# talmolab/flybody

Measured on AMD Instinct MI355X. Metric: env-steps/sec (whole node), fruitfly flight-imitation task, higher is better.
Workload: dtype f32; 1 GPU; flight_imitation (BASELINE configs[3]): 4 substeps @5e-5 s (joint limits, fluid forces, the fly's own contacts) + WBPG + obs/reward/termination/auto-reset; envs_per_gpu=8192, global_batch=8192, parallelism=env-sharded x1, actions=uniform over the raw action spec (canonical U(-1,1)), resident in HBM

## Files before the change

### flybody_amd/build.py

```python

from __future__ import annotations

import os
import subprocess

_HERE = os.path.dirname(os.path.abspath(__file__))
CSRC = os.path.join(_HERE, "csrc")
LIB = os.path.join(CSRC, "libflybody_env.so")
SOURCES = ["fly_env.hip", "ball_env.hip", "nstep.hip"]
PER_SOURCE_FLAGS = {
    "fly_env.hip": ["-mllvm", "-disable-machine-licm"],
    "ball_env.hip": ["-mllvm", "-sink-insts-to-avoid-spills=1"],
}
HEADERS = ["dev_model.hpp", "ball_model.hpp", "ball_env.hpp", "dev_math.hpp", "convex.hpp", "launch_order.hpp", os.path.join("..", "..", "include", "flybody_env.h")]


def needs_build() -> bool:
    if not os.path.exists(LIB):
        return True
    t = os.path.getmtime(LIB)
    return any(os.path.getmtime(os.path.join(CSRC, f)) > t for f in SOURCES + HEADERS)


def _common_flags() -> list:
    hipcc = os.environ.get("HIPCC", "/opt/rocm/bin/hipcc")
    common = [hipcc, "--offload-arch=gfx950", "-O3", "-std=c++17", "-fPIC", "-fno-slp-vectorize",
              "-mllvm", "-amdgpu-sched-strategy=iterative-ilp"]
    return common


def kernel_resource_usage(src: str = "fly_env.hip", match: str = "flight_step_kernel") -> dict:
    import re
    import tempfile

    with tempfile.TemporaryDirectory() as tmp:
        cmd = _common_flags() + PER_SOURCE_FLAGS.get(src, []) + ["--cuda-device-only", "-Rpass-analysis=kernel-resource-usage", "-c",
                                                                 os.path.join(CSRC, src), "-o", os.path.join(tmp, "dev.o")]
        text = subprocess.run(cmd, check=True, stderr=subprocess.PIPE, stdout=subprocess.DEVNULL, text=True).stderr
    out, cur = {}, None
    for line in text.splitlines():
        m = re.search(r"remark: Function Name: (\S+)", line)
        if m:
            cur = out.setdefault(m.group(1), {}) if match in m.group(1) else None
            continue
        m = re.search(r"remark:\s+([A-Za-z ]+?)(?: \[[^\]]*\])?: (\d+)", line)
        if m and cur is not None:
            cur[m.group(1).strip()] = int(m.group(2))
    return out


def build(force: bool = False, verbose: bool = False) -> str:
    if not force and not needs_build():
        return LIB
    common = _common_flags()
    hipcc = common[0]
    objs = []
    for src in SOURCES:
        obj = os.path.join(CSRC, "_obj_" + os.path.splitext(src)[0] + ".o")
        cmd = common + PER_SOURCE_FLAGS.get(src, []) + ["-c", os.path.join(CSRC, src), "-o", obj]
        if verbose:
            print(" ".join(cmd))
        subprocess.check_call(cmd)
        objs.append(obj)
    cmd = [hipcc, "--offload-arch=gfx950", "-shared", "-fPIC", "-o", LIB] + objs
    if verbose:
        print(" ".join(cmd))
    subprocess.check_call(cmd)
    for obj in objs:
        os.remove(obj)
    return LIB


if __name__ == "__main__":
    print(build(force=True, verbose=True))
```

### flybody_amd/csrc/fly_env.hip

```cpp
#include <hip/hip_runtime.h>

#include <cstdio>
#include <cstring>
#include <memory>
#include <string>
#include <vector>

#include "../../include/flybody_env.h"
#include "ball_env.hpp"
#include "dev_model.hpp"
#include "launch_order.hpp"
#include "dev_math.hpp"
#include "convex.hpp"

#ifndef FFE_WAVES_PER_SIMD
#define FFE_WAVES_PER_SIMD 4
#endif

namespace ffe {

constexpr int kMC = 6;
constexpr int kMCX = 12;
constexpr int kCapExit = 0x100;
constexpr int kNSD = 16;
// ... 325 lines not shown
  } while (0)
#endif
#ifdef FFE_DBGCF
__device__ float g_dbgcf[64][4 + 6 * 12];
#endif
#ifdef FFE_STAMPS
__device__ unsigned long long g_stamps[20];
#define STAMP_DECL unsigned long long st_t0 = __builtin_amdgcn_s_memtime(), st_acc[20] = {0}
#define STAMP(k)                                                   \
  do {                                                             \
    __builtin_amdgcn_s_waitcnt(0);                                 \
    unsigned long long st_t1 = __builtin_amdgcn_s_memtime();       \
    c.st_acc[k] += st_t1 - c.st_t0;                                \
    c.st_t0 = st_t1;                                               \
  } while (0)
#define CSTAMP(k)                                                                                  \
  do {                                                                                             \
    __builtin_amdgcn_s_waitcnt(0);                                                                 \
    unsigned long long cs_t1 = __builtin_amdgcn_s_memtime();                                       \
    if (lane == 0) atomicAdd(&g_stamps[k], cs_t1 - cs_t0);                                         \
    cs_t0 = cs_t1;                                                                                 \
  } while (0)
#define CSTAMP_DECL unsigned long long cs_t0 = __builtin_amdgcn_s_memtime()
#else
#define STAMP(k) do {} while (0)
#define CSTAMP(k) do {} while (0)
#define CSTAMP_DECL do {} while (0)
#endif
__device__ __forceinline__ void set_com(Ctx &c, V3 v) { if (c.lane == 0) { c.T.sens[9] = v.x; c.T.sens[10] = v.y; c.T.sens[11] = v.z; } }
__device__ __forceinline__ V3 get_com(const Ctx &c) { return {c.T.sens[9], c.T.sens[10], c.T.sens[11]}; }
#ifdef FFE_TRACE
#define TRACE_HI(c) (((unsigned)(c).nrare & 0xffu) | (((unsigned)(c).nfac & 0xffu) << 8) | ((min((c).tr_coll, 0xffffu)) << 16))
__device__ unsigned long long g_trace[32768][4];
#define TRACE_BEGIN unsigned long long tr_t0 = __builtin_amdgcn_s_memrealtime(); const int tr_prev = cost[order[blockIdx.x]]
#define TRACE_END(slot, tr_extra, tr_hi)                                                                                              \
  do {                                                                                                                         \
    __builtin_amdgcn_s_waitcnt(0);                                                                                             \
    if (threadIdx.x == 0 && (slot) < 32768) {                                                                                  \
      g_trace[slot][0] = tr_t0; g_trace[slot][1] = __builtin_amdgcn_s_memrealtime();                                               \
      g_trace[slot][2] = (unsigned long long)__builtin_amdgcn_s_getreg((31 << 11) | 4) | ((unsigned long long)tr_hi << 32);                                                 \
      g_trace[slot][3] = (__builtin_amdgcn_s_getreg((31 << 11) | 20) & 0xf) | ((unsigned long long)(tr_extra) << 8);  \
    }                                                                                                                          \
  } while (0)
#else
#define TRACE_BEGIN do {} while (0)
#define TRACE_HI(c) 0
#define TRACE_END(slot, tr_extra, tr_hi) do {} while (0)
#endif
#ifdef FFE_ABLATION
#define DBG(c, f) ((c).flags & (f))
#else
#define DBG(c, f) (0)
#endif
enum { DBG_SKIP_FACTOR = 1 << 16, DBG_SKIP_SOLVE = 1 << 17, DBG_SKIP_STAGE1 = 1 << 18, DBG_SKIP_MENTRIES = 1 << 19, DBG_SKIP_GHOST = 1 << 20, DBG_SKIP_WBPG = 1 << 21, DBG_SKIP_OBS = 1 << 22, DBG_NO_CARRY = 1 << 23, DBG_NO_ORDER = 1 << 24 };

struct CollA { float4 gc[kMaxGeom], gq[kMaxGeom]; float lq[kMaxLink][4]; float sdc[kNSD][5], sdn[kNSD][5]; };
constexpr int kCL2 = 24;
template <int MC> struct CollB { unsigned short cl1[128], cl2[kCL2]; float rec[MC][12]; float cl2n[kCL2][5]; };
static_assert(sizeof(CollA) <= sizeof(Tile::LD), "collision scratch A");
static_assert(sizeof(CollB<kMC>) == 1072 && sizeof(CollB<kMCX>) == 1360 && sizeof(CollB<kMCX>) <= sizeof(Tile::lT) + sizeof(Tile::lb) + sizeof(Tile::lc) && offsetof(Tile, lc) == offsetof(Tile, lT) + sizeof(Tile::lT) + sizeof(Tile::lb), "collision scratch B");
__device__ __forceinline__ CollA &coll_a(Tile &T) { return *reinterpret_cast<CollA *>(&T.LD[0]); }
template <int MC> __device__ __forceinline__ CollB<MC> &coll_b(Tile &T) { return *reinterpret_cast<CollB<MC> *>(&T.lT[0][0]); }

__device__ __forceinline__ cvx::Geom load_geom(const CollA &A, const DevModel FFE_CONST &M, int g) {
  const float4 cc = A.gc[g], qq = A.gq[g];
  return cvx::Geom{dm::V3{cc.x, cc.y, cc.z}, dm::Q4{qq.x, qq.y, qq.z, qq.w}, M.cg_size[g], M.cg_size[kMaxGeom + g], M.cg_size[2 * kMaxGeom + g], M.cg_type[g]};
}

__device__ __forceinline__ cvx::UShape ush(const DevModel FFE_CONST &M, int g) {
  const float4 u = M.cg_ush[2 * g], k = M.cg_ush[2 * g + 1];
  return cvx::UShape{u.x, u.y, u.z, u.w, k.x, k.y, k.z, k.w};
}

template <bool WITH_RARE, int MC>
__device__ __forceinline__ int collide_narrow(Tile &T, const DevModel FFE_CONST &M, const int lane, int n2, int nk, int ovf) {
  CollA &A = coll_a(T);
  CollB<MC> &B = coll_b<MC>(T);
  const unsigned long long mm0 = M.cg_mmask[0], mm1 = M.cg_mmask[1];
  const float mclass = M.c_margin;
  auto pair_margin = [&](int a, int b) {
    const bool ma = a < 64 ? ((mm0 >> a) & 1ull) : ((mm1 >> (a - 64)) & 1ull), mb = b < 64 ? ((mm0 >> b) & 1ull) : ((mm1 >> (b - 64)) & 1ull);
    return (ma || mb) ? mclass : 0.f;
  };
  bool hit = false;
  float dist = 0.f, margin = 0.f, ctt = 0.f;
  dm::V3 nrm = {1.f, 0.f, 0.f}, cpos = {0.f, 0.f, 0.f};
  int a = 0, b = 0;
// ... 987 lines not shown
    obs[L.gyro] = s_gyro.x; obs[L.gyro + 1] = s_gyro.y; obs[L.gyro + 2] = s_gyro.z;
    obs[L.vel] = s_vel.x; obs[L.vel + 1] = s_vel.y; obs[L.vel + 2] = s_vel.z;
    obs[L.zaxis] = T.xmat[0][6]; obs[L.zaxis + 1] = T.xmat[0][7]; obs[L.zaxis + 2] = T.xmat[0][8];
  }
  if (lane < M.nobsj) {
    obs[L.jpos + lane] = T.qpos[M.obsj_qadr[lane]];
    obs[L.jvel + lane] = T.qvel[M.obsj_dof[lane]];
  }
  float cd = 0.f;
  Q4 r0 = {1.f, 0.f, 0.f, 0.f};
  if (lane < nref) {
    const double *r = K.ref_qpos + ((size_t)traj_row0 + step_counter + lane) * 7;
    V3 dv = {(float)(r[0] - T.rootpos[0]), (float)(r[1] - T.rootpos[1]), (float)(r[2] - T.rootpos[2])};
    V3 e = mtv(ldm(T.xmat[0]), dv);
    obs[L.rdisp + 3 * lane] = e.x; obs[L.rdisp + 3 * lane + 1] = e.y; obs[L.rdisp + 3 * lane + 2] = e.z;
    Q4 fq = {T.qpos[3], T.qpos[4], T.qpos[5], T.qpos[6]};
    Q4 dq = qmul(quat_recip(fq), Q4{(float)r[3], (float)r[4], (float)r[5], (float)r[6]});
    obs[L.rquat + 4 * lane] = dq.w; obs[L.rquat + 4 * lane + 1] = dq.x; obs[L.rquat + 4 * lane + 2] = dq.y; obs[L.rquat + 4 * lane + 3] = dq.z;
    if (lane == 0) { cd = sqrtf(dot(e, e)); r0 = dq; }
  }
  com_dist = __shfl(cd, 0);
  rq0 = {__shfl(r0.w, 0), __shfl(r0.x, 0), __shfl(r0.y, 0), __shfl(r0.z, 0)};
}

__device__ __forceinline__ void load_lane_consts(Ctx &c) {
  const DevModel FFE_CONST &M = *c.Mp;
  c.dinv[0] = c.dinv[1] = 0.f;
  c.la_pack = (unsigned)M.d_madr[c.lane] | ((unsigned)M.d_depth[c.lane] << 10) | ((unsigned)M.d_ndesc[c.lane] << 16);
  c.seq0 = M.br_seq[c.lane]; c.seq1 = M.br_seq[kWave + c.lane]; c.seq2 = M.br_seq[2 * kWave + c.lane]; c.seq3 = M.br_seq[3 * kWave + c.lane];
  for (int e = c.lane; e < M.nM; e += kWave) c.T.colmadr[e] = M.colmadr[e];
}

template <int MC>
__global__ __launch_bounds__(kWave, FFE_WAVES_PER_SIMD) void flight_step_kernel(const DevModel *__restrict__ Mp_, const TaskDev *__restrict__ Kp_, typename StateOf<MC>::type *__restrict__ states, const float *__restrict__ act,
                                                              float *__restrict__ obs_out, float *__restrict__ reward_out,
                                                              float *__restrict__ discount_out, int *__restrict__ step_type_out, int batch, int mode, int nphys,
                                                              const int *__restrict__ order, int *__restrict__ cost,
                                                              const unsigned char *__restrict__ reset_mask) {
  __shared__ Tile T;
  const DevModel FFE_CONST *Mp = (const DevModel FFE_CONST *)Mp_;
  const TaskDev FFE_CONST *Kp = (const TaskDev FFE_CONST *)Kp_;
  const DevModel FFE_CONST &M = *Mp;
  const TaskDev FFE_CONST &K = *Kp;
  if ((int)blockIdx.x >= batch) return;
  TRACE_BEGIN;
  const int env = order[blockIdx.x];
  if (mode == 3) {
    if (!reset_mask[env]) return;
    mode = 1;
  }
  const int lane = threadIdx.x;
  typename StateOf<MC>::type &SX = states[env];
  EnvState &S = common(SX);
  Ctx c{Mp, T, lane, K.flags, 0.f, 0.f, {0.f, 0.f}, 0u, 0u, 0u, 0u, 0u};
#ifdef FFE_DBGCF
  c.dbg_env = env;
#endif
  c.pc = -1;
  c.nrare = 0; c.nfac = 0;
#ifdef FFE_TRACE
  c.tr_coll = 0u;
#endif
#ifdef FFE_STAMPS
  c.st_t0 = __builtin_amdgcn_s_memtime();
  for (int k = 0; k < 20; k++) c.st_acc[k] = 0;
#endif
  load_lane_consts(c);
  if (lane < kNSD) { c.sd_nx = S.sd_n[lane][0]; c.sd_ny = S.sd_n[lane][1]; c.sd_nz = S.sd_n[lane][2]; c.sd_t = S.sd_n[lane][3]; c.sd_pid = S.sd_pid[lane]; }
  c.sd_cnt = S.s1_valid ? S.sd_cnt : 0;
  float *obs = obs_out + (size_t)env * K.obs_dim;
  const bool phys_only = (mode == 2);
  const int nsub = phys_only ? nphys : M.nsub;

  if (lane < 3) T.rootpos[lane] = S.rootpos[lane];
  if (lane < 9) T.sens[lane] = 0.f;
  unsigned long long lo_mask = S.lo_mask, hi_mask = S.hi_mask, in_lo = S.in_lo_mask, in_hi = S.in_hi_mask;
  int wb_step = S.wb_step, wb_idx = S.wb_freq_idx, step_counter = S.step_counter, traj_idx = S.traj_idx;
  double wb_cf = S.wb_ctrl_freq;
  int wb_off = S.wb_off, wb_len = S.wb_len, traj_row0 = S.traj_row0;
  const bool do_reset = !phys_only && ((mode == 1) || (S.needs_reset != 0));
  int iters = 0;
  const bool have_saved = !do_reset && S.s1_valid != 0 && !DBG(c, DBG_NO_CARRY);
  constexpr int kCarry = (kMaxDof * 6 + kWave - 1) / kWave;
  float pre_c[kCarry], pre_b[kCarry], pre_f = 0.f, pre_m = 0.f;
  if (have_saved) {
#pragma unroll
    for (int k = 0; k < kCarry; k++) {
      const int e = lane + k * kWave;
      pre_c[k] = e < kMaxDof * 6 ? S.s1_cdof[e] : 0.f; pre_b[k] = e < kMaxDof * 6 ? S.s1_buf[e] : 0.f;
    }
    pre_f = S.s1_f[lane];
    pre_m = lane < 12 ? S.s1_misc[lane] : 0.f;
  }

  unsigned long long episode = S.episode;
  float ctrl_reg = 0.f;
  if (do_reset) {
    double phase;
    if (S.forced_traj >= 0) { traj_idx = S.forced_traj; phase = S.forced_phase; }
    else {
      traj_idx = (int)(env_rng(K.seed, K.env_id_base + env, episode, 0) % (unsigned long long)K.ntraj);
      phase = (double)(env_rng(K.seed, K.env_id_base + env, episode, 1) >> 11) * (1.0 / 9007199254740992.0);
    }
    episode++;
    step_counter = 0;
    wb_cf = K.base_freq;
    wb_idx = wave_argmin_absdiff(K.beat_freqs, K.nfreq, wb_cf, lane);
    int off = K.tab_off[wb_idx], len = K.tab_off[wb_idx + 1] - off;
    wb_off = off; wb_len = len;
    wb_step = wave_argmin_absdiff(K.phase + off, len, phase, lane);
    const int nxt = wb_step + 1 < len ? wb_step + 1 : 0;
    const int row0 = K.traj_off[traj_idx];
    traj_row0 = row0;
    const double *rq = K.ref_qpos + (size_t)row0 * 7, *rv = K.ref_qvel + (size_t)row0 * 6;
    if (lane < kMaxDof + 4) { T.qpos[lane] = lane < M.nq ? M.qpos0[lane] : 0.f; T.qvel[lane] = 0.f; }
    SYNC();
    if (lane == 0) {
// ... 41 lines not shown
                                             : wave_argmin_absdiff(K.beat_freqs, K.nfreq, wb_cf, lane));
      if (idx_new != wb_idx) {
        double cur = K.phase_frac[wb_off + wb_step];
        int noff = K.tab_off[idx_new], nlen = K.tab_off[idx_new + 1] - noff;
        wb_step = wave_argmin_absdiff(K.phase_frac + noff, nlen, cur, lane);
        wb_idx = idx_new; wb_off = noff; wb_len = nlen;
        if (lane < M.nwing) tgt = K.traj[(size_t)(wb_off + wb_step) * 6 + lane];
      }
    }
    STAMP(15);
    if (lane < M.nu) T.ctrl[lane] = ai >= 0 ? to_real(a_raw, ai) : 0.f;
    if (lane < 13) T.ghost[lane] = gh;
    SYNC();
    if (lane < M.nwing) {
      float add = tgt - T.qpos[M.wing_qadr[lane]];
      const int u = M.wing_ctrl[lane];
      if (u >= 0) T.ctrl[u] += add;
    }
    SYNC();
    ctrl_reg = lane < M.nu ? T.ctrl[lane] : 0.f;
    SYNC();
    step_counter++;
  }
  {
    const float abase = do_reset ? 0.f : actuation_base(c, ctrl_reg);
    if (lane < kMaxAct) T.ctrl[lane] = abase;
  }
  if (lane == 0) {
    T.park_d[0] = wb_cf; T.park_d[1] = __longlong_as_double((long long)episode);
    T.park_i[0] = wb_step; T.park_i[1] = wb_idx; T.park_i[2] = step_counter; T.park_i[3] = traj_idx; T.park_i[4] = 0; T.park_i[5] = 0;
    T.park_i[6] = S.v_ep_flagged; T.park_i[7] = S.v_ep_bits;
  }
  STAMP(11);
  const int nst = do_reset ? 1 : nsub;
#pragma unroll 1
  for (int s = 0; s <= nst; s++) {
    if (s == 0 && have_saved) {
#pragma unroll
      for (int k = 0; k < kCarry; k++) {
        const int e = lane + k * kWave;
        if (e < kMaxDof * 6) { (&T.cdof[0][0])[e] = pre_c[k]; (&T.buf[0][0])[e] = pre_b[k]; }
      }
      c.f_smooth_nb = pre_f;
      if (lane < MC) {
        const float *o = ct_f_row(SX, lane);
        c.ct_nx = o[0]; c.ct_ny = o[1]; c.ct_nz = o[2]; c.ct_px = o[3]; c.ct_py = o[4]; c.ct_pz = o[5]; c.ct_dist = o[6]; c.ct_incl = o[7]; c.ct_invw = o[8];
        const int *oi = ct_i_row(SX, lane);
        c.ct_l1 = oi[0]; c.ct_l2 = oi[1]; c.ct_pid = oi[2];
      }
      c.nct = S.nct;
      if (lane < 9) T.xmat[0][lane] = pre_m;
      else if (lane < 12) T.sens[lane] = pre_m;
      SYNC();
    } else if (!DBG(c, DBG_SKIP_STAGE1) || s == 0) { stage1(c); flight_collide<MC>(c); STAMP(16); }
    if (lane < 6 && (do_reset || s > 0)) {
      float add;
      if (lane < 3) add = T.xmat[0][lane] * T.qvel[0] + T.xmat[0][3 + lane] * T.qvel[1] + T.xmat[0][6 + lane] * T.qvel[2];
      else add = T.qvel[lane];
      T.sens[lane < 3 ? 6 + lane : lane] += add;
    }
    if (s == nst) break;
    float qa = 0.f;
    if (!do_reset) qa = actuation(c, lane < kMaxAct ? T.ctrl[lane] : 0.f);
    STAMP(12);
    int it = 0;
    const V3 acc = stage2<MC>(c, qa, !do_reset, !do_reset && !phys_only && !DBG(c, DBG_SKIP_GHOST), K.ghost_accel_z, lo_mask, hi_mask, in_lo, in_hi, it);
    if (lane == 0) { T.park_i[4] += it; if (s < 4) T.park_i[5] |= min(c.nct, 15) << (4 * s); }
    if (lane < 3) T.sens[lane] += lane == 0 ? acc.x : (lane == 1 ? acc.y : acc.z);
    if (do_reset) break;
  }
  SYNC();
  wb_cf = T.park_d[0]; episode = (unsigned long long)__double_as_longlong(T.park_d[1]);
  wb_step = T.park_i[0]; wb_idx = T.park_i[1]; step_counter = T.park_i[2]; traj_idx = T.park_i[3]; iters = T.park_i[4];
  V3 s_acc = {T.sens[0], T.sens[1], T.sens[2]}, s_gyro = {T.sens[3], T.sens[4], T.sens[5]}, s_vel = {T.sens[6], T.sens[7], T.sens[8]};
  if (!phys_only) {
  const float inv = (do_reset && K.pad_first_obs) ? 1.f : 1.f / (float)nsub;
  float cdist;
  Q4 rq0;
  const int traj_row0 = K.traj_off[traj_idx], traj_rows = K.traj_off[traj_idx + 1] - traj_row0;
  if (DBG(c, DBG_SKIP_OBS)) { cdist = 0.f; rq0 = {1.f, 0.f, 0.f, 0.f}; }
  else write_obs(c, K, obs, inv * s_acc, inv * s_gyro, inv * s_vel, traj_row0, step_counter, cdist, rq0);
  if (do_reset) {
    if (lane == 0) { reward_out[env] = 0.f; discount_out[env] = 1.f; step_type_out[env] = FFE_STEP_FIRST; S.needs_reset = 0; S.forced_traj = -1; }
  } else {
    float qn2 = wave_sum(lane < M.nv ? c.qacc * c.qacc : 0.f);
    float height = (float)T.rootpos[2];
    int lim = traj_rows < K.time_limit_steps ? traj_rows : K.time_limit_steps;
    int traj_timesteps = lim - (K.future_steps + 1);
    bool reached_end = (step_counter == traj_timesteps);
    bool bad = !(qn2 == qn2) || !(sqrtf(qn2) <= 1e14f);
    bool term = height < 0.2f || cdist > (float)K.terminal_com_dist || reached_end || bad;
    if (lane == 0) {
      const double ox = -0.03697732, oy = 0.00029205, oz = -0.0142447;
      const double *gpos = T.ghost, *rootpos = T.rootpos;
      const V3 com_e = get_com(c);
      double w = T.ghost[3], x = T.ghost[4], y = T.ghost[5], z = T.ghost[6];
      double n2 = w * w + x * x + y * y + z * z;
      double gx = gpos[0] + ((w * w + x * x - y * y - z * z) * ox + 2 * (x * y - w * z) * oy + 2 * (x * z + w * y) * oz) / n2;
      double gy = gpos[1] + (2 * (x * y + w * z) * ox + (w * w - x * x + y * y - z * z) * oy + 2 * (y * z - w * x) * oz) / n2;
      double gz = gpos[2] + (2 * (x * z - w * y) * ox + 2 * (y * z + w * x) * oy + (w * w - x * x - y * y + z * z) * oz) / n2;
      double dx = gx - (rootpos[0] + (double)com_e.x), dy = gy - (rootpos[1] + (double)com_e.y), dz = gz - (rootpos[2] + (double)com_e.z);
      float r1 = fmaxf(0.f, 1.f - (float)sqrt(dx * dx + dy * dy + dz * dz) / 0.4f);
      float r2 = fmaxf(0.f, 1.f - quat_dist_short_arc(Q4{1.f, 0.f, 0.f, 0.f}, rq0) / 3.14159265358979f);
      float reward = r1 * r2;
// ... 18 lines not shown
    S.nactive = __popcll(lo_mask) + __popcll(hi_mask);
    const int hist_c = T.park_i[5], csum = (hist_c & 15) + ((hist_c >> 4) & 15) + ((hist_c >> 8) & 15) + ((hist_c >> 12) & 15);
    const int work = min(255, (11 * c.nfac + 2 * csum + 14 * c.nrare) / 2);
    int pred = work;
    if (!phys_only) {
      const int off = K.tab_off[wb_idx], len = K.tab_off[wb_idx + 1] - off;
      const int b = min(31, (int)(K.phase_frac[off + wb_step] * 32.0));
      const int nb = min(31, (int)(K.phase_frac[off + (wb_step + 1 < len ? wb_step + 1 : 0)] * 32.0));
      if (do_reset) { for (int k = 0; k < 32; k++) S.cost_hist[k] = 0; }
      else S.cost_hist[b] = (unsigned char)work;
      pred = max(pred, max((int)S.cost_hist[nb], (int)S.cost_hist[(nb + 1) & 31]));
    }
    cost[env] = pred;
  }
  for (int e = lane; e < kMaxDof * 6; e += kWave) { S.s1_cdof[e] = (&T.cdof[0][0])[e]; S.s1_buf[e] = (&T.buf[0][0])[e]; }
  S.s1_f[lane] = c.f_smooth_nb;
  if (lane < 9) S.s1_misc[lane] = T.xmat[0][lane];
  if (lane == 0) { const V3 com_e = get_com(c); S.s1_misc[9] = com_e.x; S.s1_misc[10] = com_e.y; S.s1_misc[11] = com_e.z; S.s1_valid = 1; }
  if (lane < MC) {
    float *o = ct_f_row(SX, lane);
    o[0] = c.ct_nx; o[1] = c.ct_ny; o[2] = c.ct_nz; o[3] = c.ct_px; o[4] = c.ct_py; o[5] = c.ct_pz; o[6] = c.ct_dist; o[7] = c.ct_incl; o[8] = c.ct_invw;
    int *oi = ct_i_row(SX, lane);
    oi[0] = c.ct_l1; oi[1] = c.ct_l2; oi[2] = c.ct_pid;
  }
  if (lane < kNSD) { S.sd_n[lane][0] = c.sd_nx; S.sd_n[lane][1] = c.sd_ny; S.sd_n[lane][2] = c.sd_nz; S.sd_n[lane][3] = c.sd_t; S.sd_pid[lane] = c.sd_pid; }
  if (lane == 0) {
    S.nct = c.nct; S.sd_cnt = c.sd_cnt; S.ct_pad[0] = c.ct_ovf & 255; S.ct_pad[1] = T.park_i[5];
    const int vb = ((c.ct_ovf & 255) ? 1 : 0) | ((c.ct_ovf & kCapExit) ? 2 : 0);
    S.v_step_bits = vb;
    if (!phys_only) { S.v_ep_flagged = do_reset ? 0 : T.park_i[6] + (vb ? 1 : 0); S.v_ep_bits = do_reset ? 0 : (T.park_i[7] | vb); }
  }
#ifdef FFE_STAMPS
  STAMP(10);
  if (lane == 0) for (int k = 0; k < 20; k++) atomicAdd(&g_stamps[k], c.st_acc[k]);
#endif
  TRACE_END(blockIdx.x, (unsigned long long)((unsigned)(iters & 0xff) | ((unsigned)(__popcll(lo_mask) + __popcll(hi_mask)) << 8) | ((unsigned)(tr_prev & 0xffff) << 16)) | ((unsigned long long)(T.park_i[5] & 0xffff) << 32), TRACE_HI(c));
}

__global__ void init_states_kernel(void *states, size_t stride, int *order, int *cost, int batch) {
  int i = blockIdx.x * blockDim.x + threadIdx.x;
  if (i >= batch) return;
  EnvState z;
  memset(&z, 0, sizeof(z));
  z.needs_reset = 1; z.forced_traj = -1;
  state_at(states, stride, i) = z;
  if (stride > sizeof(EnvState)) memset(reinterpret_cast<char *>(&state_at(states, stride, i)) + sizeof(EnvState), 0, stride - sizeof(EnvState));
  order[i] = i;
  cost[i] = 0;
}

__global__ void get_state_kernel(void *states, size_t stride, double *qpos, double *qvel, int batch, int nq, int nv) {
  int env = blockIdx.x, lane = threadIdx.x;
  if (env >= batch) return;
  const EnvState &S = state_at(states, stride, env);
  if (lane < nq) qpos[(size_t)env * nq + lane] = lane < 3 ? S.rootpos[lane] : (double)S.qpos[lane];
  if (lane < nv) qvel[(size_t)env * nv + lane] = (double)S.qvel[lane];
}
__global__ void set_state_kernel(void *states, size_t stride, const double *qpos, const double *qvel, int batch, int nq, int nv) {
  int env = blockIdx.x, lane = threadIdx.x;
  if (env >= batch) return;
  EnvState &S = state_at(states, stride, env);
  if (lane < nq) { if (lane < 3) S.rootpos[lane] = qpos[(size_t)env * nq + lane]; else S.qpos[lane] = (float)qpos[(size_t)env * nq + lane]; }
  if (lane < nv) S.qvel[lane] = (float)qvel[(size_t)env * nv + lane];
  if (lane == 0) { S.lo_mask = 0; S.hi_mask = 0; S.in_lo_mask = 0; S.in_hi_mask = 0; S.s1_valid = 0; }
}
__global__ void get_task_state_kernel(void *states, size_t stride, int *ints, double *reals, int batch) {
  int i = blockIdx.x * blockDim.x + threadIdx.x;
  if (i >= batch) return;
  const EnvState &S = state_at(states, stride, i);
// ... 14 lines not shown
  if (i >= batch) return;
  state_at(states, stride, i).forced_traj = traj[i];
  state_at(states, stride, i).forced_phase = phase[i];
}
__global__ void test_quat_kernel(int op, const float *a, const float *b, float *out, int n) {
  int i = blockIdx.x * blockDim.x + threadIdx.x;
  if (i >= n) return;
  Q4 qa = {a[4 * i], a[4 * i + 1], a[4 * i + 2], a[4 * i + 3]}, qb = {b[4 * i], b[4 * i + 1], b[4 * i + 2], b[4 * i + 3]};
  Q4 r = {0, 0, 0, 0};
  if (op == 0) r = qmul(qa, qb);
  else if (op == 1) r = quat_recip(qa);
  else if (op == 2) { V3 v = rotate_vec_with_quat(V3{qa.w, qa.x, qa.y}, qb); r = {v.x, v.y, v.z, 0.f}; }
  else if (op == 3) r = {quat_dist_short_arc(qa, qb), 0.f, 0.f, 0.f};
  else if (op == 4) r = qmul(quat_recip(qa), qb);
  out[4 * i] = r.w; out[4 * i + 1] = r.x; out[4 * i + 2] = r.y; out[4 * i + 3] = r.z;
}

}

using namespace ffe;

struct ffe_env {
  ffb::BallEnv *ball = nullptr;
  int device = 0, batch = 0;
  DevModel dm{};
  TaskDev task{};
  DevModel *dm_dev = nullptr;
  TaskDev *task_dev = nullptr;
  HostModel host;
  void *states = nullptr;
  size_t state_stride = sizeof(EnvState);
  int contact_capacity = kMC;
  int *order = nullptr, *cost = nullptr;
  bool timing = false; double timing_ms = 0.0;
  unsigned char *arena = nullptr;
  std::vector<void *> allocs;
  std::string err;
  hipEvent_t ev0 = nullptr, ev1 = nullptr;
  int *forced_traj_dev = nullptr;
  double *forced_phase_dev = nullptr;
};

static thread_local std::string g_err;

struct DeviceGuard {
  int prev = -1;
  bool switched = false;
  explicit DeviceGuard(int device) {
    if (hipGetDevice(&prev) != hipSuccess) prev = -1;
    if (prev != device) { switched = (hipSetDevice(device) == hipSuccess); }
  }
  ~DeviceGuard() { if (switched && prev >= 0) (void)hipSetDevice(prev); }
  DeviceGuard(const DeviceGuard &) = delete;
  DeviceGuard &operator=(const DeviceGuard &) = delete;
};

#define HIP_OK(expr)                                                                              \
  do {                                                                                            \
    hipError_t _e = (expr);                                                                       \
    if (_e != hipSuccess) throw std::runtime_error(std::string(#expr) + ": " + hipGetErrorString(_e)); \
  } while (0)

template <typename T>
static T *upload(ffe_env *h, const T *src, size_t n) {
  T *p = nullptr;
  HIP_OK(hipMalloc(reinterpret_cast<void **>(&p), (n ? n : 1) * sizeof(T)));
// ... 86 lines not shown
    TaskDev &K = h->task;
    K.nfreq = t.wb_nfreq; K.ntraj = t.ntraj; K.future_steps = t.future_steps; K.time_limit_steps = t.time_limit_steps;
    K.episode_limit_steps = t.episode_limit_steps > 0 ? t.episode_limit_steps : t.time_limit_steps;
    K.pad_first_obs = t.pad_first_obs; K.flags = t.physics_flags; K.canonical = t.canonical_actions; K.clip = t.clip_actions;
    for (int k = 0; k < 16; k++) { K.act_lo[k] = k < h->dm.naction ? h->host.action_min[k] : 0.f; K.act_hi[k] = k < h->dm.naction ? h->host.action_max[k] : 0.f; }
    K.base_freq = t.wb_base_freq; K.rel_range = t.wb_rel_range; K.rate = t.wb_rate; K.dt_ctrl = t.wb_dt_ctrl;
    K.terminal_com_dist = t.terminal_com_dist; K.ghost_accel_z = t.ghost_accel_z;
    K.grid_inv_step = 0.0;
    if (t.wb_nfreq >= 3) {
      const double step = (t.wb_beat_freqs[t.wb_nfreq - 1] - t.wb_beat_freqs[0]) / (t.wb_nfreq - 1);
      bool even = step > 0;
      for (int i = 0; i < t.wb_nfreq && even; i++) even = std::fabs(t.wb_beat_freqs[i] - (t.wb_beat_freqs[0] + i * step)) < 0.25 * step;
      if (even) K.grid_inv_step = 1.0 / step;
    }
    set_off(K.beat_freqs, (size_t)upload(h.get(), t.wb_beat_freqs, (size_t)t.wb_nfreq));
    set_off(K.tab_off, (size_t)upload(h.get(), t.wb_tab_off, (size_t)t.wb_nfreq + 1));
    set_off(K.phase, (size_t)upload(h.get(), t.wb_phase, (size_t)rows));
    set_off(K.phase_frac, (size_t)upload(h.get(), frac.data(), frac.size()));
    set_off(K.traj, (size_t)upload(h.get(), trajf.data(), trajf.size()));
    set_off(K.ref_qpos, (size_t)upload(h.get(), t.ref_qpos, ref_rows * 7));
    set_off(K.ref_qvel, (size_t)upload(h.get(), t.ref_qvel, ref_rows * 6));
    set_off(K.traj_off, (size_t)upload(h.get(), toff.data(), toff.size()));
    K.seed = seed; K.env_id_base = env_id_base;
    K.obs_dim = 12 + 2 * h->dm.nobsj + 7 * (t.future_steps + 1);
    h->host.nobs = K.obs_dim;
    h->dm_dev = upload(h.get(), &h->dm, 1);
    h->task_dev = upload(h.get(), &h->task, 1);
    HIP_OK(hipMalloc(&h->states, h->state_stride * (size_t)batch));
    h->allocs.push_back(h->states);
    HIP_OK(hipMalloc(reinterpret_cast<void **>(&h->order), sizeof(int) * (size_t)batch));
    h->allocs.push_back(h->order);
    HIP_OK(hipMalloc(reinterpret_cast<void **>(&h->cost), sizeof(int) * (size_t)batch));
    h->allocs.push_back(h->cost);
    hipLaunchKernelGGL(init_states_kernel, dim3((batch + 255) / 256), dim3(256), 0, 0, h->states, h->state_stride, h->order, h->cost, batch);
    HIP_OK(hipGetLastError());
    HIP_OK(hipDeviceSynchronize());
    HIP_OK(hipEventCreate(&h->ev0));
    HIP_OK(hipEventCreate(&h->ev1));
  } catch (const std::exception &e) {
    g_err = e.what();
    for (void *p : h->allocs) (void)hipFree(p);
    if (h->ev0) (void)hipEventDestroy(h->ev0);
    if (h->ev1) (void)hipEventDestroy(h->ev1);
    return -1;
  }
  *out = h.release();
  return 0;
}

int ffe_destroy(ffe_handle h) {
  if (!h) return -1;
  DeviceGuard guard(h->device);
  if (h->ball) { ffb::ball_destroy(h->ball); delete h; return 0; }
  for (void *p : h->allocs) (void)hipFree(p);
  if (h->ev0) (void)hipEventDestroy(h->ev0);
  if (h->ev1) (void)hipEventDestroy(h->ev1);
  delete h;
  return 0;
}

int ffe_spec(ffe_handle h, ffe_spec_t *s) {
  if (!h || !s) return -1;
  if (h->ball) {
    std::memset(s, 0, sizeof(*s));
    ffb::ball_spec(h->ball, &s->nq, &s->nv, &s->nu, &s->action_dim, &s->obs_dim, &s->nsub, &s->physics_timestep, &s->control_timestep);
    s->batch = h->batch;
    s->off_accelerometer = 0; s->off_gyro = 104; s->off_joints_pos = 107; s->off_joints_vel = 192; s->off_velocimeter = 283; s->off_world_zaxis = 286;
    s->off_ref_displacement = -1; s->off_ref_root_quat = -1; s->n_obs_joints = 85; s->n_ref = 0;
    return 0;
  }
  const DevModel &M = h->dm;
  const int nref = h->task.future_steps + 1, nj = M.nobsj;
  s->batch = h->batch; s->nq = M.nq; s->nv = M.nv; s->nu = M.nu; s->action_dim = M.naction; s->obs_dim = h->task.obs_dim; s->nsub = M.nsub;
  s->physics_timestep = (double)M.h; s->control_timestep = h->task.dt_ctrl;
  s->off_accelerometer = 0; s->off_gyro = 3; s->off_joints_pos = 6; s->off_joints_vel = 6 + nj; s->off_velocimeter = 6 + 2 * nj;
  s->off_world_zaxis = 9 + 2 * nj; s->off_ref_displacement = 12 + 2 * nj; s->off_ref_root_quat = 12 + 2 * nj + 3 * nref;
  s->n_obs_joints = nj; s->n_ref = nref;
  return 0;
}

int ffe_action_bounds(ffe_handle h, float *mn, float *mx) {
  if (!h || !mn || !mx) return -1;
  FFE_BALL_DISPATCH(h, ffb::ball_action_bounds(h->ball, mn, mx));
  std::memcpy(mn, h->host.action_min.data(), h->host.action_min.size() * sizeof(float));
  std::memcpy(mx, h->host.action_max.data(), h->host.action_max.size() * sizeof(float));
  return 0;
}

#ifndef FFE_ORDER_MAX_BATCH
#define FFE_ORDER_MAX_BATCH 8192
#endif
static int launch_step(ffe_handle h, const float *act, float *obs, float *rew, float *disc, int32_t *st, void *stream, int mode, int nphys = 0,
                       const uint8_t *mask = nullptr) {
  if (!h) return -1;
  DeviceGuard guard(h->device);
  FFE_BALL_DISPATCH(h, ffb::ball_launch(h->ball, act, obs, rew, disc, st, stream, mode, nphys, mask));
  if (mode != 2 && (!obs || !rew || !disc || !st || (mode == 0 && !act))) { h->err = "null device buffer"; return -1; }
  if (h->timing && hipEventRecord(h->ev0, static_cast<hipStream_t>(stream)) != hipSuccess) return -2;
  if (h->contact_capacity == kMCX)
    hipLaunchKernelGGL(flight_step_kernel<kMCX>, dim3(h->batch), dim3(kWave), 0, static_cast<hipStream_t>(stream), h->dm_dev, h->task_dev, static_cast<EnvStateX *>(h->states), act,
                       obs, rew, disc, st, h->batch, mode, nphys, h->order, h->cost, mask);
  else
    hipLaunchKernelGGL(flight_step_kernel<kMC>, dim3(h->batch), dim3(kWave), 0, static_cast<hipStream_t>(stream), h->dm_dev, h->task_dev, static_cast<EnvState *>(h->states), act, obs, rew,
                       disc, st, h->batch, mode, nphys, h->order, h->cost, mask);
  hipError_t e = hipGetLastError();
  if (e != hipSuccess) { h->err = hipGetErrorString(e); return -2; }
  if (h->timing && hipEventRecord(h->ev1, static_cast<hipStream_t>(stream)) != hipSuccess) return -2;
  if (mode == 0 && h->batch > 1 && h->batch <= FFE_ORDER_MAX_BATCH && !(h->task.flags & DBG_NO_ORDER)) {
    hipLaunchKernelGGL(ffe_order::order_by_cost, dim3(1), dim3(1024), 0, static_cast<hipStream_t>(stream), h->cost, h->order, h->batch);
    e = hipGetLastError();
    if (e != hipSuccess) { h->err = hipGetErrorString(e); return -2; }
  }
  if (h->timing) {
    float t = 0.f;
    if (hipEventSynchronize(h->ev1) != hipSuccess || hipEventElapsedTime(&t, h->ev0, h->ev1) != hipSuccess) return -2;
    h->timing_ms += t;
  }
  return 0;
}

int ffe_reset(ffe_handle h, float *obs, float *rew, float *disc, int32_t *st, void *stream) { return launch_step(h, nullptr, obs, rew, disc, st, stream, 1); }
int ffe_reset_envs(ffe_handle h, const uint8_t *mask, float *obs, float *rew, float *disc, int32_t *st, void *stream) {
  if (!h) return -1;
  if (!mask) { h->err = "null reset mask"; return -1; }
  return launch_step(h, nullptr, obs, rew, disc, st, stream, 3, 0, mask);
}
int ffe_step(ffe_handle h, const float *act, float *obs, float *rew, float *disc, int32_t *st, void *stream) {
  return launch_step(h, act, obs, rew, disc, st, stream, 0);
}

int ffe_physics_step(ffe_handle h, const float *ctrl, int nsteps, void *stream) {
  if (!h || !ctrl || nsteps <= 0) return -1;
  return launch_step(h, ctrl, nullptr, nullptr, nullptr, nullptr, stream, 2, nsteps);
}

int ffe_force_next_episode(ffe_handle h, const int32_t *traj, const double *phase, void *stream) {
  if (!h || !traj || !phase) return -1;
// ... 108 lines not shown
```

### flybody_amd/csrc/launch_order.hpp

```cpp
#pragma once
#include <hip/hip_runtime.h>

namespace ffe_order {
namespace {

__global__ __launch_bounds__(1024) void order_by_cost(const int *__restrict__ cost, int *__restrict__ order, int batch) {
  __shared__ int hist[256], start[256];
  const int t = threadIdx.x;
  if (t < 256) hist[t] = 0;
  __syncthreads();
  constexpr int KPT = 16;
  int key[KPT];
#pragma unroll
  for (int q = 0; q < KPT; q++) {
    const int e = t + q * 1024;
    key[q] = e < batch ? min(255, max(0, cost[e])) : -1;
    if (key[q] >= 0) atomicAdd(&hist[key[q]], 1);
  }
  for (int e = t + KPT * 1024; e < batch; e += 1024) atomicAdd(&hist[min(255, max(0, cost[e]))], 1);
  __syncthreads();
  if (t < 256) start[t] = hist[t];
  __syncthreads();
  for (int off = 1; off < 256; off <<= 1) {
    int v = 0;
    if (t < 256 && t + off < 256) v = start[t + off];
    __syncthreads();
    if (t < 256) start[t] += v;
    __syncthreads();
  }
  if (t < 256) start[t] -= hist[t];
  __syncthreads();
#pragma unroll
  for (int q = 0; q < KPT; q++)
    if (key[q] >= 0) order[atomicAdd(&start[key[q]], 1)] = t + q * 1024;
  for (int e = t + KPT * 1024; e < batch; e += 1024) order[atomicAdd(&start[min(255, max(0, cost[e]))], 1)] = e;
}

}
}
```

Before: 11.33 million env-steps/s.

## Make step kernel persistent with atomic work queue over cost-sorted envs

```diff
diff --git a/flybody_amd/build.py b/flybody_amd/build.py
--- a/flybody_amd/build.py
+++ b/flybody_amd/build.py
@@ -29,14 +29,27 @@
     return common
 
 
+_DEVICE_COMPILES: dict = {}
+
+
+def _device_compile(src: str) -> tuple:
+    import tempfile
+
+    if src not in _DEVICE_COMPILES:
+        with tempfile.TemporaryDirectory() as tmp:
+            asm = os.path.join(tmp, "dev.s")
+            cmd = _common_flags() + PER_SOURCE_FLAGS.get(src, []) + ["--cuda-device-only", "-Rpass-analysis=kernel-resource-usage", "-S",
+                                                                     os.path.join(CSRC, src), "-o", asm]
+            remarks = subprocess.run(cmd, check=True, stderr=subprocess.PIPE, stdout=subprocess.DEVNULL, text=True).stderr
+            with open(asm) as f:
+                _DEVICE_COMPILES[src] = (remarks, f.read())
+    return _DEVICE_COMPILES[src]
+
+
 def kernel_resource_usage(src: str = "fly_env.hip", match: str = "flight_step_kernel") -> dict:
     import re
-    import tempfile
 
-    with tempfile.TemporaryDirectory() as tmp:
-        cmd = _common_flags() + PER_SOURCE_FLAGS.get(src, []) + ["--cuda-device-only", "-Rpass-analysis=kernel-resource-usage", "-c",
-                                                                 os.path.join(CSRC, src), "-o", os.path.join(tmp, "dev.o")]
-        text = subprocess.run(cmd, check=True, stderr=subprocess.PIPE, stdout=subprocess.DEVNULL, text=True).stderr
+    text = _device_compile(src)[0]
     out, cur = {}, None
     for line in text.splitlines():
         m = re.search(r"remark: Function Name: (\S+)", line)
@@ -46,6 +59,21 @@
         m = re.search(r"remark:\s+([A-Za-z ]+?)(?: \[[^\]]*\])?: (\d+)", line)
         if m and cur is not None:
             cur[m.group(1).strip()] = int(m.group(2))
+    return out
+
+
+def kernel_arg_layout(src: str = "fly_env.hip", match: str = "flight_step_kernel") -> dict:
+    import re
+
+    meta = _device_compile(src)[1]
+    meta = meta[meta.index("amdhsa.kernels:"):]
+    out = {}
+    for block in meta.split("  - .agpr_count:")[1:]:
+        names = re.findall(r"^    \.name:\s+(\S+)", block, re.M)
+        if not names or match not in names[0]:
+            continue
+        args = re.findall(r"\.offset:\s+(\d+)\s+\.size:\s+(\d+)\s+\.value_kind:\s+(\w+)", block)
+        out[names[0]] = [(int(o), int(sz)) for o, sz, kind in args if not kind.startswith("hidden")]
     return out
 
 
diff --git a/flybody_amd/csrc/fly_env.hip b/flybody_amd/csrc/fly_env.hip
--- a/flybody_amd/csrc/fly_env.hip
+++ b/flybody_amd/csrc/fly_env.hip
@@ -381,7 +381,7 @@
 #ifdef FFE_TRACE
 #define TRACE_HI(c) (((unsigned)(c).nrare & 0xffu) | (((unsigned)(c).nfac & 0xffu) << 8) | ((min((c).tr_coll, 0xffffu)) << 16))
 __device__ unsigned long long g_trace[32768][4];
-#define TRACE_BEGIN unsigned long long tr_t0 = __builtin_amdgcn_s_memrealtime(); const int tr_prev = cost[order[blockIdx.x]]
+#define TRACE_BEGIN(key) unsigned long long tr_t0 = __builtin_amdgcn_s_memrealtime(); const int tr_prev = (key)
 #define TRACE_END(slot, tr_extra, tr_hi)                                                                                              \
   do {                                                                                                                         \
     __builtin_amdgcn_s_waitcnt(0);                                                                                             \
@@ -392,7 +392,7 @@
     }                                                                                                                          \
   } while (0)
 #else
-#define TRACE_BEGIN do {} while (0)
+#define TRACE_BEGIN(key) do {} while (0)
 #define TRACE_HI(c) 0
 #define TRACE_END(slot, tr_extra, tr_hi) do {} while (0)
 #endif
@@ -401,7 +401,8 @@
 #else
 #define DBG(c, f) (0)
 #endif
-enum { DBG_SKIP_FACTOR = 1 << 16, DBG_SKIP_SOLVE = 1 << 17, DBG_SKIP_STAGE1 = 1 << 18, DBG_SKIP_MENTRIES = 1 << 19, DBG_SKIP_GHOST = 1 << 20, DBG_SKIP_WBPG = 1 << 21, DBG_SKIP_OBS = 1 << 22, DBG_NO_CARRY = 1 << 23, DBG_NO_ORDER = 1 << 24 };
+enum { DBG_SKIP_FACTOR = 1 << 16, DBG_SKIP_SOLVE = 1 << 17, DBG_SKIP_STAGE1 = 1 << 18, DBG_SKIP_MENTRIES = 1 << 19, DBG_SKIP_GHOST = 1 << 20, DBG_SKIP_WBPG = 1 << 21, DBG_SKIP_OBS = 1 << 22, DBG_NO_CARRY = 1 << 23, DBG_NO_ORDER = 1 << 24,
+       DBG_ONE_PER_ENV = 1 << 25 };
 
 struct CollA { float4 gc[kMaxGeom], gq[kMaxGeom]; float lq[kMaxLink][4]; float sdc[kNSD][5], sdn[kNSD][5]; };
 constexpr int kCL2 = 24;
@@ -1455,25 +1456,58 @@
 }
 
 template <int MC>
+struct StepArgs {
+  const DevModel FFE_GLOBAL *Mp; const TaskDev FFE_GLOBAL *Kp; typename StateOf<MC>::type FFE_GLOBAL *states; const float FFE_GLOBAL *act;
+  float FFE_GLOBAL *obs_out; float FFE_GLOBAL *reward_out; float FFE_GLOBAL *discount_out; int FFE_GLOBAL *step_type_out;
+  int batch, mode, nphys;
+  const int FFE_GLOBAL *order; int FFE_GLOBAL *cost; const unsigned char FFE_GLOBAL *reset_mask; unsigned FFE_GLOBAL *queue;
+};
+static_assert(offsetof(StepArgs<kMC>, obs_out) == 32 && offsetof(StepArgs<kMC>, batch) == 64 && offsetof(StepArgs<kMC>, nphys) == 72 &&
+              offsetof(StepArgs<kMC>, order) == 80 && offsetof(StepArgs<kMC>, queue) == 104 && sizeof(StepArgs<kMC>) == 112, "kernarg layout");
+template <int MC>
+__device__ __forceinline__ const StepArgs<MC> FFE_CONST &step_args() {
+#if defined(__HIP_DEVICE_COMPILE__)
+  const StepArgs<MC> FFE_CONST *a = (const StepArgs<MC> FFE_CONST *)__builtin_amdgcn_kernarg_segment_ptr();
+  asm volatile("" : "+s"(a));
+  return *a;
+#else
+  return *(const StepArgs<MC> *)nullptr;
+#endif
+}
+template <int MC>
 __global__ __launch_bounds__(kWave, FFE_WAVES_PER_SIMD) void flight_step_kernel(const DevModel *__restrict__ Mp_, const TaskDev *__restrict__ Kp_, typename StateOf<MC>::type *__restrict__ states, const float *__restrict__ act,
                                                               float *__restrict__ obs_out, float *__restrict__ reward_out,
                                                               float *__restrict__ discount_out, int *__restrict__ step_type_out, int batch, int mode, int nphys,
                                                               const int *__restrict__ order, int *__restrict__ cost,
-                                                              const unsigned char *__restrict__ reset_mask) {
+                                                              const unsigned char *__restrict__ reset_mask, unsigned *__restrict__ queue) {
   __shared__ Tile T;
-  const DevModel FFE_CONST *Mp = (const DevModel FFE_CONST *)Mp_;
-  const TaskDev FFE_CONST *Kp = (const TaskDev FFE_CONST *)Kp_;
+  if ((int)blockIdx.x >= batch) {
+    ffe_order::pulled_position(queue, ffe_order::pull(queue, threadIdx.x == 0), batch, threadIdx.x == 0);
+    return;
+  }
+#ifdef FFE_STAMPS
+  unsigned long long st_sum[20] = {0};
+#endif
+  int pos = blockIdx.x, lane = threadIdx.x;
+#pragma unroll 1
+  do {
+  const StepArgs<MC> FFE_CONST &A = step_args<MC>();
+  const DevModel FFE_CONST *Mp = (const DevModel FFE_CONST *)A.Mp;
+  const TaskDev FFE_CONST *Kp = (const TaskDev FFE_CONST *)A.Kp;
+  asm volatile("" : "+s"(Mp), "+s"(Kp));
+  asm volatile("" : "+v"(lane));
   const DevModel FFE_CONST &M = *Mp;
   const TaskDev FFE_CONST &K = *Kp;
-  if ((int)blockIdx.x >= batch) return;
-  TRACE_BEGIN;
-  const int env = order[blockIdx.x];
+  const unsigned pull_v = ffe_order::pull_issue((unsigned *)A.queue, lane == 0);
+  const int env = A.order[pos];
+  TRACE_BEGIN(A.cost[env]);
+  int mode = A.mode;
   if (mode == 3) {
-    if (!reset_mask[env]) return;
+    if (!A.reset_mask[env]) { pos = ffe_order::pulled_position((unsigned *)A.queue, ffe_order::pull_take(pull_v), A.batch, lane == 0); continue; }
     mode = 1;
   }
-  const int lane = threadIdx.x;
-  typename StateOf<MC>::type &SX = states[env];
+  const float *act = (const float *)A.act;
+  typename StateOf<MC>::type &SX = ((typename StateOf<MC>::type *)A.states)[env];
   EnvState &S = common(SX);
   Ctx c{Mp, T, lane, K.flags, 0.f, 0.f, {0.f, 0.f}, 0u, 0u, 0u, 0u, 0u};
 #ifdef FFE_DBGCF
@@ -1491,9 +1525,8 @@
   load_lane_consts(c);
   if (lane < kNSD) { c.sd_nx = S.sd_n[lane][0]; c.sd_ny = S.sd_n[lane][1]; c.sd_nz = S.sd_n[lane][2]; c.sd_t = S.sd_n[lane][3]; c.sd_pid = S.sd_pid[lane]; }
   c.sd_cnt = S.s1_valid ? S.sd_cnt : 0;
-  float *obs = obs_out + (size_t)env * K.obs_dim;
   const bool phys_only = (mode == 2);
-  const int nsub = phys_only ? nphys : M.nsub;
+  const int nsub = phys_only ? A.nphys : M.nsub;
 
   if (lane < 3) T.rootpos[lane] = S.rootpos[lane];
   if (lane < 9) T.sens[lane] = 0.f;
@@ -1506,6 +1539,8 @@
   const bool have_saved = !do_reset && S.s1_valid != 0 && !DBG(c, DBG_NO_CARRY);
   constexpr int kCarry = (kMaxDof * 6 + kWave - 1) / kWave;
   float pre_c[kCarry], pre_b[kCarry], pre_f = 0.f, pre_m = 0.f;
+#pragma unroll
+  for (int k = 0; k < kCarry; k++) pre_c[k] = pre_b[k] = 0.f;
   if (have_saved) {
 #pragma unroll
     for (int k = 0; k < kCarry; k++) {
@@ -1613,6 +1648,7 @@
     T.park_i[6] = S.v_ep_flagged; T.park_i[7] = S.v_ep_bits;
   }
   STAMP(11);
+  const unsigned pull_n = ffe_order::pull_take(pull_v);
   const int nst = do_reset ? 1 : nsub;
 #pragma unroll 1
   for (int s = 0; s <= nst; s++) {
@@ -1651,6 +1687,9 @@
     if (do_reset) break;
   }
   SYNC();
+  const StepArgs<MC> FFE_CONST &E = step_args<MC>();
+  float *reward_out = (float *)E.reward_out, *discount_out = (float *)E.discount_out, *obs = (float *)E.obs_out + (size_t)env * K.obs_dim;
+  int *step_type_out = (int *)E.step_type_out, *cost = (int *)E.cost;
   wb_cf = T.park_d[0]; episode = (unsigned long long)__double_as_longlong(T.park_d[1]);
   wb_step = T.park_i[0]; wb_idx = T.park_i[1]; step_counter = T.park_i[2]; traj_idx = T.park_i[3]; iters = T.park_i[4];
   V3 s_acc = {T.sens[0], T.sens[1], T.sens[2]}, s_gyro = {T.sens[3], T.sens[4], T.sens[5]}, s_vel = {T.sens[6], T.sens[7], T.sens[8]};
@@ -1735,9 +1774,14 @@
   }
 #ifdef FFE_STAMPS
   STAMP(10);
-  if (lane == 0) for (int k = 0; k < 20; k++) atomicAdd(&g_stamps[k], c.st_acc[k]);
+  for (int k = 0; k < 20; k++) st_sum[k] += c.st_acc[k];
 #endif
-  TRACE_END(blockIdx.x, (unsigned long long)((unsigned)(iters & 0xff) | ((unsigned)(__popcll(lo_mask) + __popcll(hi_mask)) << 8) | ((unsigned)(tr_prev & 0xffff) << 16)) | ((unsigned long long)(T.park_i[5] & 0xffff) << 32), TRACE_HI(c));
+  TRACE_END(pos, (unsigned long long)((unsigned)(iters & 0xff) | ((unsigned)(__popcll(lo_mask) + __popcll(hi_mask)) << 8) | ((unsigned)(tr_prev & 0xffff) << 16)) | ((unsigned long long)(T.park_i[5] & 0xffff) << 32), TRACE_HI(c));
+  pos = ffe_order::pulled_position((unsigned *)E.queue, pull_n, E.batch, lane == 0);
+  } while (pos >= 0);
+#ifdef FFE_STAMPS
+  if (lane == 0) for (int k = 0; k < 20; k++) atomicAdd(&g_stamps[k], st_sum[k]);
+#endif
 }
 
 __global__ void init_states_kernel(void *states, size_t stride, int *order, int *cost, int batch) {
@@ -1818,6 +1862,8 @@
   size_t state_stride = sizeof(EnvState);
   int contact_capacity = kMC;
   int *order = nullptr, *cost = nullptr;
+  unsigned *queue = nullptr;
+  int grid = 0;
   bool timing = false; double timing_ms = 0.0;
   unsigned char *arena = nullptr;
   std::vector<void *> allocs;
@@ -1970,6 +2016,18 @@
     h->allocs.push_back(h->order);
     HIP_OK(hipMalloc(reinterpret_cast<void **>(&h->cost), sizeof(int) * (size_t)batch));
     h->allocs.push_back(h->cost);
+    HIP_OK(hipMalloc(reinterpret_cast<void **>(&h->queue), sizeof(unsigned)));
+    h->allocs.push_back(h->queue);
+    HIP_OK(hipMemset(h->queue, 0, sizeof(unsigned)));
+    {
+      int per_cu = 0;
+      hipDeviceProp_t prop;
+      HIP_OK(hipGetDeviceProperties(&prop, device));
+      if (h->contact_capacity == kMCX) HIP_OK(hipOccupancyMaxActiveBlocksPerMultiprocessor(&per_cu, flight_step_kernel<kMCX>, kWave, 0));
+      else HIP_OK(hipOccupancyMaxActiveBlocksPerMultiprocessor(&per_cu, flight_step_kernel<kMC>, kWave, 0));
+      if (per_cu < 1) throw std::runtime_error("ffe_create_flight: the step kernel does not fit a compute unit");
+      h->grid = ffe_order::step_grid(batch, per_cu * prop.multiProcessorCount, (t.physics_flags & DBG_ONE_PER_ENV) != 0);
+    }
     hipLaunchKernelGGL(init_states_kernel, dim3((batch + 255) / 256), dim3(256), 0, 0, h->states, h->state_stride, h->order, h->cost, batch);
     HIP_OK(hipGetLastError());
     HIP_OK(hipDeviceSynchronize());
@@ -2036,11 +2094,11 @@
   if (mode != 2 && (!obs || !rew || !disc || !st || (mode == 0 && !act))) { h->err = "null device buffer"; return -1; }
   if (h->timing && hipEventRecord(h->ev0, static_cast<hipStream_t>(stream)) != hipSuccess) return -2;
   if (h->contact_capacity == kMCX)
-    hipLaunchKernelGGL(flight_step_kernel<kMCX>, dim3(h->batch), dim3(kWave), 0, static_cast<hipStream_t>(stream), h->dm_dev, h->task_dev, static_cast<EnvStateX *>(h->states), act,
-                       obs, rew, disc, st, h->batch, mode, nphys, h->order, h->cost, mask);
+    hipLaunchKernelGGL(flight_step_kernel<kMCX>, dim3(h->grid), dim3(kWave), 0, static_cast<hipStream_t>(stream), h->dm_dev, h->task_dev, static_cast<EnvStateX *>(h->states), act,
+                       obs, rew, disc, st, h->batch, mode, nphys, h->order, h->cost, mask, h->queue);
   else
-    hipLaunchKernelGGL(flight_step_kernel<kMC>, dim3(h->batch), dim3(kWave), 0, static_cast<hipStream_t>(stream), h->dm_dev, h->task_dev, static_cast<EnvState *>(h->states), act, obs, rew,
-                       disc, st, h->batch, mode, nphys, h->order, h->cost, mask);
+    hipLaunchKernelGGL(flight_step_kernel<kMC>, dim3(h->grid), dim3(kWave), 0, static_cast<hipStream_t>(stream), h->dm_dev, h->task_dev, static_cast<EnvState *>(h->states), act, obs, rew,
+                       disc, st, h->batch, mode, nphys, h->order, h->cost, mask, h->queue);
   hipError_t e = hipGetLastError();
   if (e != hipSuccess) { h->err = hipGetErrorString(e); return -2; }
   if (h->timing && hipEventRecord(h->ev1, static_cast<hipStream_t>(stream)) != hipSuccess) return -2;
diff --git a/flybody_amd/csrc/launch_order.hpp b/flybody_amd/csrc/launch_order.hpp
--- a/flybody_amd/csrc/launch_order.hpp
+++ b/flybody_amd/csrc/launch_order.hpp
@@ -1,5 +1,6 @@
 #pragma once
 #include <hip/hip_runtime.h>
+#include <cstdlib>
 
 namespace ffe_order {
 namespace {
@@ -36,5 +37,28 @@
   for (int e = t + KPT * 1024; e < batch; e += 1024) order[atomicAdd(&start[min(255, max(0, cost[e]))], 1)] = e;
 }
 
+__device__ __forceinline__ unsigned pull_issue(unsigned *counter, bool leader) {
+  unsigned v = 0u;
+  if (leader) v = __hip_atomic_fetch_add(counter, 1u, __ATOMIC_RELAXED, __HIP_MEMORY_SCOPE_AGENT);
+  return v;
+}
+__device__ __forceinline__ unsigned pull_take(unsigned v) { return (unsigned)__builtin_amdgcn_readfirstlane((int)v); }
+__device__ __forceinline__ unsigned pull(unsigned *counter, bool leader) { return pull_take(pull_issue(counter, leader)); }
+__device__ __forceinline__ int pulled_position(unsigned *counter, unsigned v, int batch, bool leader) {
+  const unsigned npull = max((unsigned)batch, (unsigned)gridDim.x);
+  if (v == npull - 1u && leader) __hip_atomic_store(counter, 0u, __ATOMIC_RELAXED, __HIP_MEMORY_SCOPE_AGENT);
+  const unsigned p = v + (unsigned)gridDim.x;
+  return p < (unsigned)batch ? (int)p : -1;
+}
+
+}
+
+inline int step_grid(int batch, int resident, bool one_per_env) {
+  int grid = one_per_env ? batch : (batch < resident ? batch : resident);
+  if (const char *s = getenv("FLYBODY_STEP_GRID")) {
+    const long n = strtol(s, nullptr, 10);
+    if (n >= 1) grid = (int)(n < (1L << 30) ? n : (1L << 30));
+  }
+  return grid < 1 ? 1 : grid;
 }
 }
```

New measurement: 10.38 million env-steps/s. 8.4% lower.
